# dspcraft/dsc

Measured on AMD Instinct MI355X. Metric: batched 1-D rfft GSamples/s, higher is better.
Workload: dtype f32

## Files before the change

### dsc_amd/csrc/fft_r2c_64k.hip

```cpp
#include "kernels.h"

#include <hip/hip_runtime.h>

#include <cmath>
#include <cstdlib>
#include <utility>

namespace {

typedef float f2 __attribute__((ext_vector_type(2)));

struct cf { float x, y; };
__device__ __forceinline__ cf operator+(cf a, cf b) { return cf{a.x + b.x, a.y + b.y}; }
__device__ __forceinline__ cf operator-(cf a, cf b) { return cf{a.x - b.x, a.y - b.y}; }
__device__ __forceinline__ cf to_cf(f2 a) { return cf{a.x, a.y}; }
__device__ __forceinline__ f2 to_f2(cf a) { return f2{a.x, a.y}; }

constexpr int kM = 32768;
constexpr int kPlaneFloats = 1024 * 34;
constexpr int kLdsBytes = kPlaneFloats * 4 + 1024 * 8;
constexpr int kTabEntries = 1024;

constexpr int kAuxW1024 = 0, kAuxW32768 = 1024, kAuxW65536 = 2048, kAuxEntries = 3072;

__host__ __device__ constexpr int br5(int x) {
    return ((x & 1) << 4) | ((x & 2) << 2) | (x & 4) | ((x & 8) >> 2) | ((x & 16) >> 4);
}

__device__ constexpr float kCos64[17] = {
    1.0f, 0.99518472667219688624f, 0.98078528040323044913f, 0.95694033573220886494f,
    0.92387953251128675613f, 0.88192126434835502971f, 0.83146961230254523708f, 0.77301045336273696081f,
    0.70710678118654752440f, 0.63439328416364549822f, 0.55557023301960222474f, 0.47139673682599764856f,
    0.38268343236508977173f, 0.29028467725446236764f, 0.19509032201612826785f, 0.09801714032956060199f,
    0.0f};

__device__ constexpr float root64_re(int q) {
    q &= 63;
    return q <= 16 ? kCos64[q] : q <= 32 ? -kCos64[32 - q] : q <= 48 ? -kCos64[q - 32] : kCos64[64 - q];
}
__device__ constexpr float root64_im(int q) {
    q &= 63;
    return q <= 16 ? -kCos64[16 - q] : q <= 32 ? -kCos64[q - 16] : q <= 48 ? kCos64[48 - q] : kCos64[q - 48];
}

__device__ __forceinline__ cf cmul(cf a, cf w) {
    return cf{a.x * w.x - a.y * w.y, a.x * w.y + a.y * w.x};
}
__device__ __forceinline__ cf cmul_conj(cf a, cf w) {
    return cf{a.x * w.x + a.y * w.y, a.y * w.x - a.x * w.y};
}

template<bool INV>
__device__ __forceinline__ cf twiddle_mul_second_fused(cf a, cf w) {
    if (INV) return cf{__builtin_fmaf(a.y, w.y, a.x * w.x), __builtin_fmaf(-a.x, w.y, a.y * w.x)};
    return cf{__builtin_fmaf(-a.y, w.y, a.x * w.x), __builtin_fmaf(a.y, w.x, a.x * w.y)};
}

template<bool INV, int M, int K>
__device__ __forceinline__ cf mul_root(cf d) {
    constexpr float c8 = 0.70710678118654752440f;
    if constexpr (K == 0) {
        return d;
    } else if constexpr (4 * K == M) {
        return INV ? cf{-d.y, d.x} : cf{d.y, -d.x};
    } else if constexpr (8 * K == M) {
        return INV ? cf{(d.x - d.y) * c8, (d.x + d.y) * c8} : cf{(d.x + d.y) * c8, (d.y - d.x) * c8};
    } else if constexpr (8 * K == 3 * M) {
        return INV ? cf{-(d.x + d.y) * c8, (d.x - d.y) * c8} : cf{(d.y - d.x) * c8, -(d.x + d.y) * c8};
    } else {
        constexpr float wr = root64_re(K * (64 / M));
        constexpr float wi = INV ? -root64_im(K * (64 / M)) : root64_im(K * (64 / M));
        return cf{d.x * wr - d.y * wi, d.x * wi + d.y * wr};
    }
}

#ifdef DSC_DFT32_DIF
template<bool INV, int M, int G, int... K>
__device__ __forceinline__ void dif_group(cf (&v)[32], std::integer_sequence<int, K...>) {
    (([&] {
         const cf u = v[G + K] + v[G + K + M / 2];
         const cf d = v[G + K] - v[G + K + M / 2];
         v[G + K] = u;
         v[G + K + M / 2] = mul_root<INV, M, K>(d);
     }()),
     ...);
}

template<bool INV, int M, int... G>
__device__ __forceinline__ void dif_stage(cf (&v)[32], std::integer_sequence<int, G...>) {
    (dif_group<INV, M, G * M>(v, std::make_integer_sequence<int, M / 2>{}), ...);
}

template<bool INV>
__device__ __forceinline__ void dft32(cf (&v)[32]) {
    dif_stage<INV, 32>(v, std::make_integer_sequence<int, 1>{});
    dif_stage<INV, 16>(v, std::make_integer_sequence<int, 2>{});
    dif_stage<INV, 8>(v, std::make_integer_sequence<int, 4>{});
    dif_stage<INV, 4>(v, std::make_integer_sequence<int, 8>{});
    dif_stage<INV, 2>(v, std::make_integer_sequence<int, 16>{});
}

template<bool INV>
__device__ __forceinline__ void dft32_head(cf (&v)[32]) {
    dif_stage<INV, 32>(v, std::make_integer_sequence<int, 1>{});
    dif_stage<INV, 16>(v, std::make_integer_sequence<int, 2>{});
}
template<bool INV, int Q>
__device__ __forceinline__ void dft32_quarter(cf (&v)[32]) {
    dif_stage<INV, 8>(v, std::integer_sequence<int, Q>{});
    dif_stage<INV, 4>(v, std::integer_sequence<int, 2 * Q, 2 * Q + 1>{});
    dif_stage<INV, 2>(v, std::integer_sequence<int, 4 * Q, 4 * Q + 1, 4 * Q + 2, 4 * Q + 3>{});
}

#else
constexpr double kCos64d[17] = {
    1.0, 0.99518472667219688624, 0.98078528040323044913, 0.95694033573220886494,
    0.92387953251128675613, 0.88192126434835502971, 0.83146961230254523708, 0.77301045336273696081,
    0.70710678118654752440, 0.63439328416364549822, 0.55557023301960222474, 0.47139673682599764856,
    0.38268343236508977173, 0.29028467725446236764, 0.19509032201612826785, 0.09801714032956060199,
    0.0};

template<bool INV, int E>
__device__ __forceinline__ void dit_butterfly(cf &a, cf &b) {
    if constexpr (E == 0) {
        const cf u = a + b, d = a - b;
        a = u; b = d;
    } else if constexpr (E == 8) {
        const cf u = INV ? cf{a.x - b.y, a.y + b.x} : cf{a.x + b.y, a.y - b.x};
        const cf d = INV ? cf{a.x + b.y, a.y - b.x} : cf{a.x - b.y, a.y + b.x};
        a = u; b = d;
    } else {
        constexpr double c = E <= 8 ? kCos64d[2 * E] : -kCos64d[32 - 2 * E];
        constexpr double sn = (E <= 8 ? kCos64d[16 - 2 * E] : kCos64d[2 * E - 16]);
        constexpr double s = INV ? sn : -sn;
        if constexpr ((c < 0 ? -c : c) >= sn) {
            constexpr float t = (float) (s / c), cc = (float) c;
            float p, q;
            if constexpr (t == 1.0f) { p = b.x - b.y; q = b.y + b.x; }
            else if constexpr (t == -1.0f) { p = b.x + b.y; q = b.y - b.x; }
            else { p = __builtin_fmaf(-t, b.y, b.x); q = __builtin_fmaf(t, b.x, b.y); }
            const cf u = cf{__builtin_fmaf(cc, p, a.x), __builtin_fmaf(cc, q, a.y)};
            const cf d = cf{__builtin_fmaf(-cc, p, a.x), __builtin_fmaf(-cc, q, a.y)};
            a = u; b = d;
        } else {
            constexpr float r = (float) (c / s), ss = (float) s;
            const float pn = __builtin_fmaf(-r, b.x, b.y);
            const float q = __builtin_fmaf(r, b.y, b.x);
            const cf u = cf{__builtin_fmaf(-ss, pn, a.x), __builtin_fmaf(ss, q, a.y)};
            const cf d = cf{__builtin_fmaf(ss, pn, a.x), __builtin_fmaf(-ss, q, a.y)};
            a = u; b = d;
        }
    }
}

constexpr int brev_bits(int x, int bits) {
    int r = 0;
    for (int i = 0; i < bits; ++i) r |= ((x >> i) & 1) << (bits - 1 - i);
    return r;
}

template<bool INV, int S, int G, int... J>
__device__ __forceinline__ void dit_group(cf (&v)[32], std::integer_sequence<int, J...>) {
    constexpr int H = 32 >> S;
    constexpr int E = brev_bits(G, S - 1) * (16 >> (S - 1));
    (dit_butterfly<INV, E>(v[2 * H * G + J], v[2 * H * G + J + H]), ...);
}

template<bool INV, int S, int... G>
__device__ __forceinline__ void dit_stage(cf (&v)[32], std::integer_sequence<int, G...>) {
    (dit_group<INV, S, G>(v, std::make_integer_sequence<int, (32 >> S)>{}), ...);
}

template<bool INV>
__device__ __forceinline__ void dft32(cf (&v)[32]) {
    dit_stage<INV, 1>(v, std::make_integer_sequence<int, 1>{});
    dit_stage<INV, 2>(v, std::make_integer_sequence<int, 2>{});
    dit_stage<INV, 3>(v, std::make_integer_sequence<int, 4>{});
    dit_stage<INV, 4>(v, std::make_integer_sequence<int, 8>{});
    dit_stage<INV, 5>(v, std::make_integer_sequence<int, 16>{});
}

template<bool INV>
__device__ __forceinline__ void dft32_head(cf (&v)[32]) {
    dit_stage<INV, 1>(v, std::make_integer_sequence<int, 1>{});
    dit_stage<INV, 2>(v, std::make_integer_sequence<int, 2>{});
}
template<bool INV, int Q>
__device__ __forceinline__ void dft32_quarter(cf (&v)[32]) {
    dit_stage<INV, 3>(v, std::integer_sequence<int, Q>{});
    dit_stage<INV, 4>(v, std::integer_sequence<int, 2 * Q, 2 * Q + 1>{});
    dit_stage<INV, 5>(v, std::integer_sequence<int, 4 * Q, 4 * Q + 1, 4 * Q + 2, 4 * Q + 3>{});
}
#endif

typedef unsigned int u2 __attribute__((ext_vector_type(2)));
typedef unsigned int u4 __attribute__((ext_vector_type(4)));
typedef float f4 __attribute__((ext_vector_type(4)));

#ifndef DSC_LDS_SPLIT_READS
#define DSC_LDS_SPLIT_READS 1
#endif
__device__ __forceinline__ f2 lds_read_b64(const f2 *p) {
#if DSC_LDS_SPLIT_READS
    return *(const volatile __attribute__((address_space(3))) f2 *) p;
#else
    return *p;
#endif
}

__device__ __forceinline__ void lds_barrier() {
    __builtin_amdgcn_fence(__ATOMIC_RELEASE, "workgroup", "local");
    __builtin_amdgcn_s_barrier();
    __builtin_amdgcn_fence(__ATOMIC_ACQUIRE, "workgroup", "local");
}

__device__ __forceinline__ float bperm(int byte_addr, float x) {
    return __int_as_float(__builtin_amdgcn_ds_bpermute(byte_addr, __float_as_int(x)));
}

__device__ __forceinline__ int column_of(int wave, int lane) {
    int kp = lane < 32 ? 32 * wave + lane : 1024 - 32 * wave - (63 - lane);
    return kp == 1024 ? 512 : kp;
}

#ifdef DSC_R2C64K_PROBE
#define PROBE_ARGS , int io_on
#define PROBE_NULL , 1
#define IO_ON io_on
#else
#define PROBE_ARGS
#define PROBE_NULL
#define IO_ON 1
#endif

__device__ __forceinline__ int thread_id(int wave_sgpr) {
    int zero;
    asm volatile("v_mov_b32 %0, 0" : "=v"(zero));
    const int lane = __builtin_amdgcn_mbcnt_hi(-1, __builtin_amdgcn_mbcnt_lo(-1, zero));
    return (wave_sgpr << 6) | lane;
}

#ifndef DSC_STREAM_AUX
#define DSC_STREAM_AUX 2
#endif
constexpr int kStream = DSC_STREAM_AUX;
__device__ __forceinline__ cf load_c(__amdgpu_buffer_rsrc_t r, int voff, int soff) {
    return to_cf(__builtin_bit_cast(f2, __builtin_amdgcn_raw_buffer_load_b64(r, voff, soff, kStream)));
}
#ifndef DSC_FILTER_EARLY_LOADS
#define DSC_FILTER_EARLY_LOADS 4
#endif
#ifndef DSC_IRFFT_PIN_PASS3
#define DSC_IRFFT_PIN_PASS3 1
#endif
#ifndef DSC_IRFFT_EARLY_PAIRS
#define DSC_IRFFT_EARLY_PAIRS 4
#endif
#ifndef DSC_IRFFT_LOAD_AUX
#define DSC_IRFFT_LOAD_AUX 0
#endif
__device__ __forceinline__ cf load_c_spec(__amdgpu_buffer_rsrc_t r, int voff, int soff) {
    return to_cf(__builtin_bit_cast(f2, __builtin_amdgcn_raw_buffer_load_b64(r, voff, soff, DSC_IRFFT_LOAD_AUX)));
}
__device__ __forceinline__ cf load_c_cached(__amdgpu_buffer_rsrc_t r, int voff, int soff) {
    return to_cf(__builtin_bit_cast(f2, __builtin_amdgcn_raw_buffer_load_b64(r, voff, soff, 0)));
}
template<int POLICY>
__device__ __forceinline__ void store_c(cf a, __amdgpu_buffer_rsrc_t r, int voff, int soff) {
    __builtin_amdgcn_raw_buffer_store_b64(__builtin_bit_cast(u2, to_f2(a)), r, voff, soff, POLICY);
}

__device__ __forceinline__ void fill_twiddle_table(f2 *T, const f2 *aux) {
    const int t = threadIdx.x;
    T[t] = aux[kAuxW1024 + (t >> 5) * (t & 31)];
    __syncthreads();
}

constexpr int kCPitch = 33;
static_assert(512 * kCPitch * 8 <= kPlaneFloats * 4, "the step buffer lives inside the plane");

__host__ __device__ constexpr int class_of(int k) { return (k ^ (k >> 1)) & 1; }
__host__ __device__ constexpr int index_in_class(int k) { return ((k >> 2) << 1) | (k & 1); }
static_assert(class_of(br5(0)) == 0 && class_of(br5(7)) == 0 && class_of(br5(24)) == 0 && class_of(br5(31)) == 0 &&
              class_of(br5(8)) == 1 && class_of(br5(23)) == 1, "class 0 = quarters 0 and 3 of a dft32 output");

__device__ __forceinline__ int reader_column(int t) {
    const int a = t >> 5;
    return (t & 31) | ((((a >> 3) | ((a & 7) << 2))) << 5);
}
__device__ __forceinline__ int spectrum_wave(int wave_sgpr) { return (wave_sgpr >> 2) | ((wave_sgpr & 3) << 2); }

template<int Q>
__device__ __forceinline__ void quarter_write(f2 *buf, int wbase, const cf (&v)[32]) {
    int wbase_hi = wbase + 8 * (32 * kCPitch);
    asm("" : "+v"(wbase_hi));
    f2 *lo8 = buf + wbase;
    f2 *hi8 = buf + wbase_hi;
#pragma unroll
    for (int p = 8 * Q; p < 8 * Q + 8; ++p)
        if (index_in_class(br5(p)) < 8) lo8[index_in_class(br5(p)) * (32 * kCPitch)] = to_f2(v[p]);
#pragma unroll
    for (int p = 8 * Q; p < 8 * Q + 8; ++p)
        if (index_in_class(br5(p)) >= 8) hi8[(index_in_class(br5(p)) - 8) * (32 * kCPitch)] = to_f2(v[p]);
}

__device__ __forceinline__ void step_read(const f2 *buf, int row, cf (&dst)[32]) {
    const f2 *r = buf + __mul24(row, kCPitch);
#pragma unroll
    for (int m = 0; m < 32; ++m) dst[m] = to_cf(lds_read_b64(r + m));
}

__device__ __forceinline__ void pin(cf (&v)[32]) {
#pragma unroll
    for (int p = 0; p < 32; p += 8)
        asm volatile("" : "+v"(v[p].x), "+v"(v[p].y), "+v"(v[p + 1].x), "+v"(v[p + 1].y), "+v"(v[p + 2].x), "+v"(v[p + 2].y), "+v"(v[p + 3].x),
                     "+v"(v[p + 3].y), "+v"(v[p + 4].x), "+v"(v[p + 4].y), "+v"(v[p + 5].x), "+v"(v[p + 5].y), "+v"(v[p + 6].x), "+v"(v[p + 6].y),
                     "+v"(v[p + 7].x), "+v"(v[p + 7].y));
}

template<typename Finish>
__device__ __forceinline__ void exchange(f2 *buf, int wbase, int rclass, int rrow, cf (&src)[32], cf (&dst)[32], Finish finish) {
    pin(src);
    lds_barrier();
    finish(std::integral_constant<int, 0>{});
    quarter_write<0>(buf, wbase, src);
    finish(std::integral_constant<int, 3>{});
    quarter_write<3>(buf, wbase, src);
    lds_barrier();
    cf r[32];
    if (rclass == 0) step_read(buf, rrow, r);
    finish(std::integral_constant<int, 1>{});
    lds_barrier();
    quarter_write<1>(buf, wbase, src);
    finish(std::integral_constant<int, 2>{});
    quarter_write<2>(buf, wbase, src);
    lds_barrier();
    if (rclass != 0) step_read(buf, rrow, r);
#pragma unroll
    for (int m = 0; m < 32; ++m) dst[m] = r[m];
}

struct no_hook { __device__ __forceinline__ void operator()() const {} };

template<bool INV, typename Hook = no_hook>
__device__ __forceinline__ void three_passes(cf (&v)[32], float *plane, const f2 *T, const f2 *aux, int wave_sgpr, int col_wave,
                                             bool mirrored_in, bool mirrored_out, Hook before_pass3 = Hook{}) {
    f2 *buf = (f2 *) plane;
    const int wave_class = ((wave_sgpr >> 2) ^ (wave_sgpr >> 3)) & 1;
    dft32_head<INV>(v);
    cf u[32];
    {
        const int t = thread_id(wave_sgpr);
        const int col = mirrored_in ? column_of(col_wave, t & 63) : t;
        const int hi = col >> 5;
        const f2 *th = T + hi;
        const int rc = reader_column(t);
        exchange(buf, __mul24(col & 31, kCPitch) + hi, wave_class, (index_in_class(rc >> 5) << 5) | (rc & 31), v, u, [&](auto Q) {
            constexpr int kQ = decltype(Q)::value;
            dft32_quarter<INV, kQ>(v);
#pragma unroll
            for (int p = 8 * kQ; p < 8 * kQ + 8; ++p) {
                if (p == 0) continue;
                const cf w = to_cf(th[32 * br5(p)]);
                v[p] = INV ? cmul_conj(v[p], w) : cmul(v[p], w);
            }
        });
    }
    dft32_head<INV>(u);
    {
        const int t = thread_id(wave_sgpr);
        const int rc = reader_column(t);
        const int hi = rc >> 5, lo = rc & 31;
        const cf tw2_base = to_cf(aux[kAuxW32768 + __mul24(hi, lo)]);
        const f2 *tl = T + lo;
        const int col_out = mirrored_out ? column_of(col_wave, t & 63) : rc;
        const int k2 = col_out >> 5;
        const int rclass = mirrored_out ? class_of(k2) : wave_class;
        exchange(buf, __mul24(hi, kCPitch) + lo, rclass, (index_in_class(k2) << 5) | (col_out & 31), u, v, [&](auto Q) {
            constexpr int kQ = decltype(Q)::value;
            dft32_quarter<INV, kQ>(u);
#ifdef DSC_DFT32_DIF
            constexpr bool kSumsOnly = false;
#else
            constexpr bool kSumsOnly = true;
#endif
#pragma unroll
            for (int p = 8 * kQ; p < 8 * kQ + 8; ++p) {
                const cf w = p == 0 ? tw2_base : cmul(tw2_base, to_cf(tl[32 * br5(p)]));
                if (kSumsOnly && p < 4) u[p] = twiddle_mul_second_fused<INV>(u[p], w);
                else u[p] = INV ? cmul_conj(u[p], w) : cmul(u[p], w);
            }
        });
    }
    before_pass3();
    dft32<INV>(v);
}

__device__ __forceinline__ void real_pair(cf p, cf q, cf wq, float hs, cf &out_k, cf &out_mk) {
    const cf s = cf{p.x + q.x, p.y - q.y};
    const cf d = cf{p.x - q.x, p.y + q.y};
    const cf wd = cmul(d, wq);
    out_k = cf{hs * s.x + wd.x, hs * s.y + wd.y};
    out_mk = cf{hs * s.x - wd.x, wd.y - hs * s.y};
}

__device__ __forceinline__ int partner_byte_addr(int wave, int lane) {
    return ((wave == 0 && (lane == 63 || lane == 0)) ? lane : 63 - lane) * 4;
}

#ifndef DSC_R2C64K_HELPERS_ONLY
__global__ __launch_bounds__(1024) void rfft64k_kernel(const float *__restrict__ x, f2 *__restrict__ X, int batch,
                                                       const f2 *__restrict__ aux, int in_pitch, int in_len PROBE_ARGS) {
    extern __shared__ __attribute__((aligned(16))) float lds[];
    float *plane = lds;
    f2 *T = (f2 *) (lds + kPlaneFloats);
    fill_twiddle_table(T, aux);

    const int wave_sgpr = __builtin_amdgcn_readfirstlane(threadIdx.x >> 6);

    cf v[32];
    {
        const int row0 = blockIdx.x;
        const __amdgpu_buffer_rsrc_t r0 = __builtin_amdgcn_make_buffer_rsrc(
            (void *) (x + (size_t) row0 * in_pitch), 0, row0 < batch ? in_len * 4 * IO_ON : 0, 0x00020000);
        const int load_off = thread_id(wave_sgpr) * 8;
#pragma unroll
        for (int j1 = 0; j1 < 32; ++j1) v[j1] = load_c(r0, load_off, j1 * 8192);
    }

    for (int row = blockIdx.x; row < batch; row += gridDim.x) {
        const int next_row = row + gridDim.x;
        const __amdgpu_buffer_rsrc_t rnext = __builtin_amdgcn_make_buffer_rsrc(
            (void *) (x + (size_t) next_row * in_pitch), 0, next_row < batch ? in_len * 4 * IO_ON : 0, 0x00020000);
        const __amdgpu_buffer_rsrc_t rout =
            __builtin_amdgcn_make_buffer_rsrc((void *) (X + (size_t) row * (kM + 1)), 0, (kM + 1) * 8 * IO_ON, 0x00020000);

        const int cw = spectrum_wave(wave_sgpr);
        three_passes<false>(v, plane, T, aux, wave_sgpr, cw, false, true);

        const int t4 = thread_id(wave_sgpr);
        const int lane = t4 & 63, wave = t4 >> 6;
        const int kp = column_of(cw, lane);
        const int partner_addr = partner_byte_addr(cw, lane);
        cf xk[16], xm[16];
        const cf zmid = v[br5(16)];
        if (cw == 0) {
#pragma unroll
            for (int r = 16; r < 31; ++r) v[br5(r)] = lane == 0 ? v[br5(r + 1)] : v[br5(r)];
            v[br5(31)] = lane == 0 ? v[br5(0)] : v[br5(31)];
        }
#pragma unroll
        for (int k3 = 0; k3 < 16; ++k3) {
            const int src = 31 - br5(k3);
            xm[k3].x = bperm(partner_addr, v[src].x);
            xm[k3].y = bperm(partner_addr, v[src].y);
        }
        {
            const cf wpost = to_cf(aux[kAuxW65536 + kp]);
            const cf post_base = cf{0.5f * wpost.y, -0.5f * wpost.x};
#pragma unroll
            for (int k3 = 0; k3 < 16; ++k3) {
                const cf c = cf{root64_re(k3), root64_im(k3)};
                const cf w = k3 == 0 ? post_base : cmul(post_base, c);
                real_pair(v[br5(k3)], xm[k3], w, 0.5f, xk[k3], xm[k3]);
            }
        }

        f2 *stage = (f2 *) plane;
        const int skew = (int) ((((size_t) (X + (size_t) row * (kM + 1))) >> 3) & 15);
        lds_barrier();
#pragma unroll
        for (int k3 = 0; k3 < 16; ++k3) stage[kp + 1024 * k3] = to_f2(xk[k3]);
        const cf xk15 = xk[15];
        const int load_off = thread_id(wave_sgpr) * 8;
#pragma unroll
        for (int j1 = 0; j1 < 16; ++j1) v[j1] = load_c(rnext, load_off, j1 * 8192);
        lds_barrier();
#pragma unroll
        for (int m = 0; m < 8; ++m) {
            const int k = 2 * (t4 + 1024 * m) - skew;
            if (m > 0 || k >= 0) {
                const f2 lo2 = lds_read_b64(stage + k), hi2 = lds_read_b64(stage + k + 1);
                const f4 q = f4{lo2.x, lo2.y, hi2.x, hi2.y};
                __builtin_amdgcn_raw_buffer_store_b128(__builtin_bit_cast(u4, q), rout, k * 8, 0, kStream);
            } else if (m == 0 && k == -1) {
                __builtin_amdgcn_raw_buffer_store_b64(__builtin_bit_cast(u2, stage[0]), rout, 0, 0, kStream);
            }
            if (m & 1) __builtin_amdgcn_sched_barrier(0);
        }
        lds_barrier();
        constexpr int kStage2 = kM / 2 - 16;
#pragma unroll
        for (int k3 = 0; k3 < 16; ++k3) stage[(kM - kStage2) - kp - 1024 * k3] = to_f2(xm[k3]);
        if (kp >= 1009) stage[kp + 15 * 1024 - kStage2] = to_f2(xk15);
        if (t4 == 0) stage[kM / 2 - kStage2] = f2{zmid.x, -zmid.y};
#pragma unroll
        for (int j1 = 16; j1 < 32; ++j1) v[j1] = load_c(rnext, load_off, j1 * 8192);
        lds_barrier();
#pragma unroll
        for (int m = 0; m < 9; ++m) {
            if (m == 8 && wave != 0) break;
            const int k = kM / 2 + 2 * (t4 + 1024 * m) - skew;
            if (m < 8 || k + 1 <= kM) {
                const f2 lo2 = lds_read_b64(stage + k - kStage2), hi2 = lds_read_b64(stage + k + 1 - kStage2);
                const f4 q = f4{lo2.x, lo2.y, hi2.x, hi2.y};
                __builtin_amdgcn_raw_buffer_store_b128(__builtin_bit_cast(u4, q), rout, k * 8, 0, kStream);
            } else if (m == 8 && k == kM) {
                __builtin_amdgcn_raw_buffer_store_b64(__builtin_bit_cast(u2, stage[k - kStage2]), rout, k * 8, 0, kStream);
            }
            if (m & 1) __builtin_amdgcn_sched_barrier(0);
        }
    }
}

#endif

__device__ __forceinline__ void inverse_prepass_direct(cf (&v)[32], cf y_mid, const f2 *aux, int wave_sgpr) {
    constexpr float kScale = 1.0f / (float) kM;
    const int t1 = thread_id(wave_sgpr);
    const int lane = t1 & 63, wave = t1 >> 6;
    const int c = column_of(wave, lane);
    const int partner_addr = partner_byte_addr(wave, lane);
    if (wave == 0 && lane == 0) { v[0].y = 0.f; v[16].y = 0.f; }
    const cf wpre = to_cf(aux[kAuxW65536 + c]);
    const cf wq_base = cf{0.5f * kScale * wpre.y, 0.5f * kScale * wpre.x};
#pragma unroll
    for (int half = 0; half < 2; ++half) {
        cf zm[8];
#pragma unroll
        for (int i = 0; i < 8; ++i) {
            const int a = half * 8 + i;
            const cf cj = cf{root64_re(a), -root64_im(a)};
            const cf wq = a == 0 ? wq_base : cmul(wq_base, cj);
            real_pair(v[a], v[16 + a], wq, 0.5f * kScale, v[a], zm[i]);
        }
#pragma unroll
        for (int i = 0; i < 8; ++i) {
            const int a = half * 8 + i;
            v[16 + a].x = bperm(partner_addr, zm[i].x);
            v[16 + a].y = bperm(partner_addr, zm[i].y);
        }
    }
    cf w[32];
#pragma unroll
    for (int r = 0; r < 16; ++r) { w[r] = v[r]; w[16 + r] = v[31 - r]; }
    if (wave == 0) {
#pragma unroll
        for (int r = 31; r > 16; --r) w[r] = lane == 0 ? w[r - 1] : w[r];
        w[16] = lane == 0 ? cf{kScale * y_mid.x, -kScale * y_mid.y} : w[16];
    }
#pragma unroll
    for (int r = 0; r < 32; ++r) v[r] = w[r];
}

template<typename IssueNext>
__device__ __forceinline__ void staged_time_store(cf (&v)[32], float *plane, __amdgpu_buffer_rsrc_t rout, int wave_sgpr,
                                                  IssueNext issue_next) {
    f2 *stage = (f2 *) plane;
    const int t4 = thread_id(wave_sgpr);
    const int c4 = reader_column(t4);
    lds_barrier();
#pragma unroll
    for (int p = 0; p < 32; p += 2) stage[c4 + 1024 * br5(p)] = to_f2(v[p]);
    issue_next(true);
    lds_barrier();
#pragma unroll
    for (int m = 0; m < 8; ++m) {
        const int k = 2 * (t4 + 1024 * m);
        const f2 lo2 = lds_read_b64(stage + k), hi2 = lds_read_b64(stage + k + 1);
        const f4 q = f4{lo2.x, lo2.y, hi2.x, hi2.y};
        __builtin_amdgcn_raw_buffer_store_b128(__builtin_bit_cast(u4, q), rout, k * 8, 0, kStream);
        if (m & 1) __builtin_amdgcn_sched_barrier(0);
    }
    lds_barrier();
#pragma unroll
    for (int p = 1; p < 32; p += 2) stage[c4 + 1024 * (br5(p) - 16)] = to_f2(v[p]);
    issue_next(false);
    lds_barrier();
#pragma unroll
    for (int m = 0; m < 8; ++m) {
        const int k = 2 * (t4 + 1024 * m);
        const f2 lo2 = lds_read_b64(stage + k), hi2 = lds_read_b64(stage + k + 1);
        const f4 q = f4{lo2.x, lo2.y, hi2.x, hi2.y};
        __builtin_amdgcn_raw_buffer_store_b128(__builtin_bit_cast(u4, q), rout, (kM / 2 + k) * 8, 0, kStream);
        if (m & 1) __builtin_amdgcn_sched_barrier(0);
    }
}

__device__ __forceinline__ void unzip_rows(cf (&v)[32]) {
    cf nxt[32];
#pragma unroll
    for (int a = 0; a < 16; ++a) { nxt[a] = v[2 * a]; nxt[16 + a] = v[2 * a + 1]; }
#pragma unroll
    for (int a = 0; a < 32; ++a) v[a] = nxt[a];
}

#ifndef DSC_R2C64K_HELPERS_ONLY
__global__ __launch_bounds__(1024) void irfft64k_kernel(const f2 *__restrict__ X, float *__restrict__ x, int batch,
                                                        const f2 *__restrict__ aux, int in_pitch, int in_len PROBE_ARGS) {
    extern __shared__ __attribute__((aligned(16))) float lds[];
    float *plane = lds;
    f2 *T = (f2 *) (lds + kPlaneFloats);
    fill_twiddle_table(T, aux);

    const int wave_sgpr = __builtin_amdgcn_readfirstlane(threadIdx.x >> 6);

    cf v[32];
    cf y_mid = cf{0.f, 0.f};
    {
        const int row0 = blockIdx.x;
        const __amdgpu_buffer_rsrc_t r0 = __builtin_amdgcn_make_buffer_rsrc(
            (void *) (X + (size_t) row0 * in_pitch), 0, row0 < batch ? in_len * 8 * IO_ON : 0, 0x00020000);
        const int t0 = thread_id(wave_sgpr);
        const int c = column_of(t0 >> 6, t0 & 63);
        const int pv = (kM - c - 15 * 1024) * 8;
#pragma unroll
        for (int a = 0; a < 16; ++a) {
            v[a] = load_c_spec(r0, c * 8, a * 8192);
            v[16 + a] = load_c_spec(r0, pv, (15 - a) * 8192);
        }
        if (c == 0) y_mid = load_c_spec(r0, (kM / 2) * 8, 0);
    }

    for (int row = blockIdx.x; row < batch; row += gridDim.x) {
        const int next_row = row + gridDim.x;
        const __amdgpu_buffer_rsrc_t rnext = __builtin_amdgcn_make_buffer_rsrc(
            (void *) (X + (size_t) next_row * in_pitch), 0, next_row < batch ? in_len * 8 * IO_ON : 0, 0x00020000);
        const __amdgpu_buffer_rsrc_t rout =
            __builtin_amdgcn_make_buffer_rsrc((void *) (x + (size_t) row * 65536), 0, 65536 * 4 * IO_ON, 0x00020000);

        inverse_prepass_direct(v, y_mid, aux, wave_sgpr);
        constexpr int kEarly = DSC_IRFFT_EARLY_PAIRS;
        cf early[kEarly > 0 ? 2 * kEarly : 1];
        three_passes<true>(v, plane, T, aux, wave_sgpr, wave_sgpr, true, false, [&]() {
            if constexpr (kEarly > 0) {
                const int t3 = thread_id(wave_sgpr);
                const int c3 = column_of(t3 >> 6, t3 & 63);
                const int pv3 = (kM - c3 - 15 * 1024) * 8;
#pragma unroll
                for (int a = 0; a < kEarly; ++a) {
                    early[2 * a] = load_c_spec(rnext, c3 * 8, a * 8192);
                    early[2 * a + 1] = load_c_spec(rnext, pv3, (15 - a) * 8192);
                }
            }
        });

#if DSC_IRFFT_PIN_PASS3
#pragma unroll
        for (int p = 0; p < 32; p += 8)
            asm volatile("" : "+v"(v[p].x), "+v"(v[p].y), "+v"(v[p + 1].x), "+v"(v[p + 1].y), "+v"(v[p + 2].x), "+v"(v[p + 2].y), "+v"(v[p + 3].x),
                         "+v"(v[p + 3].y), "+v"(v[p + 4].x), "+v"(v[p + 4].y), "+v"(v[p + 5].x), "+v"(v[p + 5].y), "+v"(v[p + 6].x), "+v"(v[p + 6].y),
                         "+v"(v[p + 7].x), "+v"(v[p + 7].y));
#endif
        const int t4 = thread_id(wave_sgpr);
        const int c = column_of(t4 >> 6, t4 & 63);
        const int pv = (kM - c - 15 * 1024) * 8;
        staged_time_store(v, plane, rout, wave_sgpr, [&](bool first_half) {
            if (first_half) {
                y_mid = cf{0.f, 0.f};
                if (c == 0) y_mid = load_c_spec(rnext, (kM / 2) * 8, 0);
#pragma unroll
                for (int i = 0; i < 8; ++i) {
                    v[2 * i] = load_c_spec(rnext, c * 8, (kEarly + i) * 8192);
                    v[16 + 2 * i] = load_c_spec(rnext, pv, (15 - kEarly - i) * 8192);
                }
            } else {
#pragma unroll
                for (int i = 0; i < 8 - kEarly; ++i) {
                    v[2 * i + 1] = load_c_spec(rnext, c * 8, (kEarly + 8 + i) * 8192);
                    v[17 + 2 * i] = load_c_spec(rnext, pv, (7 - kEarly - i) * 8192);
                }
            }
        });
        {
            cf nxt[32];
#pragma unroll
            for (int a = 0; a < 16; ++a) {
                if (a < kEarly)          { nxt[a] = early[2 * a];             nxt[16 + a] = early[2 * a + 1]; }
                else if (a < kEarly + 8) { nxt[a] = v[2 * (a - kEarly)];      nxt[16 + a] = v[16 + 2 * (a - kEarly)]; }
                else                     { nxt[a] = v[2 * (a - kEarly - 8) + 1]; nxt[16 + a] = v[17 + 2 * (a - kEarly - 8)]; }
            }
#pragma unroll
            for (int a = 0; a < 32; ++a) v[a] = nxt[a];
        }
    }
}

__global__ __launch_bounds__(1024) void filter64k_kernel(const float *__restrict__ x, const f2 *__restrict__ H,
                                                         float *__restrict__ y, int batch, const f2 *__restrict__ aux, int in_pitch,
                                                         int in_len) {
    extern __shared__ __attribute__((aligned(16))) float lds[];
    float *plane = lds;
    f2 *T = (f2 *) (lds + kPlaneFloats);
    fill_twiddle_table(T, aux);

    const int wave_sgpr = __builtin_amdgcn_readfirstlane(threadIdx.x >> 6);
    const __amdgpu_buffer_rsrc_t rh = __builtin_amdgcn_make_buffer_rsrc((void *) H, 0, (kM + 1) * 8, 0x00020000);
    constexpr float kScale = 1.0f / (float) kM;

    cf v[32];
    {
        const int row0 = blockIdx.x;
        const __amdgpu_buffer_rsrc_t r0 = __builtin_amdgcn_make_buffer_rsrc(
            (void *) (x + (size_t) row0 * in_pitch), 0, row0 < batch ? in_len * 4 : 0, 0x00020000);
        const int load_off = thread_id(wave_sgpr) * 8;
#pragma unroll
        for (int j1 = 0; j1 < 32; ++j1) v[j1] = load_c(r0, load_off, j1 * 8192);
    }
    for (int row = blockIdx.x; row < batch; row += gridDim.x) {
        const int next_row = row + gridDim.x;
        const __amdgpu_buffer_rsrc_t rnext = __builtin_amdgcn_make_buffer_rsrc(
            (void *) (x + (size_t) next_row * in_pitch), 0, next_row < batch ? in_len * 4 : 0, 0x00020000);
        const __amdgpu_buffer_rsrc_t rout =
            __builtin_amdgcn_make_buffer_rsrc((void *) (y + (size_t) row * 65536), 0, 65536 * 4, 0x00020000);
        const int cw = spectrum_wave(wave_sgpr);
        three_passes<false>(v, plane, T, aux, wave_sgpr, cw, false, true);

        {
            const int t1 = thread_id(wave_sgpr);
            const int lane = t1 & 63, wave = cw;
            const int c = column_of(wave, lane);
            const int partner_addr = partner_byte_addr(wave, lane);
            const cf wc = to_cf(aux[kAuxW65536 + c]);
            const cf post_base = cf{0.5f * wc.y, -0.5f * wc.x};
            const cf pre_base = cf{0.5f * kScale * wc.y, 0.5f * kScale * wc.x};
            if (wave == 0) {
                const cf zmid = v[br5(16)];
                const cf hmid = load_c_cached(rh, (kM / 2) * 8, 0);
                const cf pmid = cmul(cf{zmid.x, -zmid.y}, hmid);
                v[br5(16)] = lane == 0 ? cf{kScale * pmid.x, -kScale * pmid.y} : v[br5(16)];
            }
            cf park = v[br5(16)];
            if (wave == 0) {
#pragma unroll
                for (int r = 16; r < 31; ++r) v[br5(r)] = lane == 0 ? v[br5(r + 1)] : v[br5(r)];
                v[br5(31)] = lane == 0 ? v[br5(0)] : v[br5(31)];
            }
#pragma unroll
            for (int part = 0; part < 8; ++part) {
                cf q[2], zm[2];
#pragma unroll
                for (int i = 0; i < 2; ++i) {
                    const int a = part * 2 + i;
                    q[i].x = bperm(partner_addr, v[br5(31 - a)].x);
                    q[i].y = bperm(partner_addr, v[br5(31 - a)].y);
                }
#pragma unroll
                for (int i = 0; i < 2; ++i) {
                    const int a = part * 2 + i;
                    const cf w64 = cf{root64_re(a), root64_im(a)};
                    cf xk, xm;
                    real_pair(v[br5(a)], q[i], a == 0 ? post_base : cmul(post_base, w64), 0.5f, xk, xm);
                    const cf hk = load_c_cached(rh, c * 8, a * 8192);
                    const cf hm = load_c_cached(rh, (kM - 15 * 1024 - c) * 8, (15 - a) * 8192);
                    cf pk = cmul(xk, hk), pm = cmul(xm, hm);
                    if (a == 0) {
                        pk.y = (c == 0) ? 0.f : pk.y;
                        pm.y = (c == 0) ? 0.f : pm.y;
                    }
                    const cf w64c = cf{root64_re(a), -root64_im(a)};
                    real_pair(pk, pm, a == 0 ? pre_base : cmul(pre_base, w64c), 0.5f * kScale, v[br5(a)], zm[i]);
                }
#pragma unroll
                for (int i = 0; i < 2; ++i) {
                    const int a = part * 2 + i;
                    v[br5(31 - a)].x = bperm(partner_addr, zm[i].x);
                    v[br5(31 - a)].y = bperm(partner_addr, zm[i].y);
                }
                __builtin_amdgcn_sched_barrier(0);
            }
            if (wave == 0) {
#pragma unroll
                for (int r = 31; r > 16; --r) v[br5(r)] = lane == 0 ? v[br5(r - 1)] : v[br5(r)];
                v[br5(16)] = lane == 0 ? park : v[br5(16)];
            }
        }
        cf z[32];
#pragma unroll
        for (int r = 0; r < 32; ++r) z[r] = v[br5(r)];
        constexpr int kEarlyX = DSC_FILTER_EARLY_LOADS;
        cf early[kEarlyX > 0 ? kEarlyX : 1];
        three_passes<true>(z, plane, T, aux, wave_sgpr, cw, true, false, [&]() {
            if constexpr (kEarlyX > 0) {
                const int off = thread_id(wave_sgpr) * 8;
#pragma unroll
                for (int j1 = 0; j1 < kEarlyX; ++j1) early[j1] = load_c(rnext, off, j1 * 8192);
            }
        });
        {
            const int load_off = thread_id(wave_sgpr) * 8;
            staged_time_store(z, plane, rout, wave_sgpr, [&](bool first_half) {
                if (first_half) {
#pragma unroll
                    for (int i = 0; i < 16; ++i) z[2 * i] = load_c(rnext, load_off, (kEarlyX + i) * 8192);
                } else {
#pragma unroll
                    for (int i = 0; i < 16 - kEarlyX; ++i) z[2 * i + 1] = load_c(rnext, load_off, (kEarlyX + 16 + i) * 8192);
                }
            });
#pragma unroll
            for (int j1 = 0; j1 < 32; ++j1) v[j1] = j1 < kEarlyX ? early[j1] : j1 < kEarlyX + 16 ? z[2 * (j1 - kEarlyX)] : z[2 * (j1 - kEarlyX - 16) + 1];
        }
    }
}

#endif

}

#ifndef DSC_R2C64K_HELPERS_ONLY
size_t dsc_r2c64k_table_bytes() { return (size_t) kAuxEntries * sizeof(float) * 2; }

void dsc_r2c64k_build_tables(void *host_dst) {
    float *o = (float *) host_dst;
    auto put = [&](int at, long long k, long long n) {
        const long double a = -2.0L * 3.14159265358979323846264338327950288L * (long double) k / (long double) n;
        o[2 * at] = (float) cosl(a);
        o[2 * at + 1] = (float) sinl(a);
    };
    for (int m = 0; m < kTabEntries; ++m) {
        put(kAuxW1024 + m, m, 1024);
        put(kAuxW32768 + m, m, 32768);
        put(kAuxW65536 + m, m, 65536);
    }
    o[2 * (kAuxW1024 + 256)] = 0.f;  o[2 * (kAuxW1024 + 256) + 1] = -1.f;
    o[2 * (kAuxW1024 + 512)] = -1.f; o[2 * (kAuxW1024 + 512) + 1] = 0.f;
    o[2 * (kAuxW1024 + 768)] = 0.f;  o[2 * (kAuxW1024 + 768) + 1] = 1.f;
}

void dsc_launch_rfft64k(const float *x, void *X, int batch, int in_pitch, int in_len, const void *aux, int n_cu, hipStream_t stream) {
    if (batch <= 0) return;
    static unsigned long long attr_devices = 0;
    if (dsc_first_use_on_device(attr_devices)) {
        DSC_KERNEL_CHECK(hipFuncSetAttribute((const void *) rfft64k_kernel, hipFuncAttributeMaxDynamicSharedMemorySize, kLdsBytes));
    }
    const int grid = batch < n_cu ? batch : n_cu;
    DSC_LAUNCH(rfft64k_kernel, dim3(grid), dim3(1024), kLdsBytes, stream, x, (f2 *) X, batch, (const f2 *) aux, in_pitch, in_len PROBE_NULL);
}

void dsc_launch_irfft64k(const void *X, float *x, int batch, int in_pitch, int in_len, const void *aux, int n_cu, hipStream_t stream) {
    if (batch <= 0) return;
    static unsigned long long attr_devices = 0;
    if (dsc_first_use_on_device(attr_devices)) {
        DSC_KERNEL_CHECK(hipFuncSetAttribute((const void *) irfft64k_kernel, hipFuncAttributeMaxDynamicSharedMemorySize, kLdsBytes));
    }
    const int grid = batch < n_cu ? batch : n_cu;
    DSC_LAUNCH(irfft64k_kernel, dim3(grid), dim3(1024), kLdsBytes, stream, (const f2 *) X, x, batch, (const f2 *) aux, in_pitch, in_len PROBE_NULL);
}
void dsc_launch_filter64k(const float *s, const void *H, float *y, int batch, int in_pitch, int in_len, const void *aux, int n_cu,
                          hipStream_t stream) {
    if (batch <= 0) return;
    static unsigned long long attr_devices = 0;
    if (dsc_first_use_on_device(attr_devices)) {
        DSC_KERNEL_CHECK(hipFuncSetAttribute((const void *) filter64k_kernel, hipFuncAttributeMaxDynamicSharedMemorySize, kLdsBytes));
    }
    const int grid = batch < n_cu ? batch : n_cu;
    DSC_LAUNCH(filter64k_kernel, dim3(grid), dim3(1024), kLdsBytes, stream, s, (const f2 *) H, y, batch, (const f2 *) aux, in_pitch, in_len);
}
#endif
```

Before: 674.4.

## Restructure rfft64k post-processing to interleave real-pair math with staged stores

Reorganizes the forward rfft epilogue so the output is staged in two phases by spectral region: the first eight real-pair outputs (both k and mirror halves) are written to LDS and streamed out while the remaining eight real pairs are computed interleaved with the LDS reads and global stores. Next-row prefetch loads go into a separate nx array and are copied into v at the end, and the real-pair computation uses explicit FMAs with a fused twiddle helper. The intent is to overlap ALU work with store traffic and cut one exposed barrier phase, at the cost of higher register pressure (extra 32-entry buffer) and complex boundary handling in the staging layout.

```diff
diff --git a/dsc_amd/csrc/fft_r2c_64k.hip b/dsc_amd/csrc/fft_r2c_64k.hip
--- a/dsc_amd/csrc/fft_r2c_64k.hip
+++ b/dsc_amd/csrc/fft_r2c_64k.hip
@@ -250,6 +250,12 @@
 #ifndef DSC_FILTER_EARLY_LOADS
 #define DSC_FILTER_EARLY_LOADS 4
 #endif
+#ifndef DSC_RFFT_EARLY_LOADS
+#define DSC_RFFT_EARLY_LOADS 16
+#endif
+#ifndef DSC_RFFT_FREE_AFTER_PAIRS
+#define DSC_RFFT_FREE_AFTER_PAIRS 0
+#endif
 #ifndef DSC_IRFFT_PIN_PASS3
 #define DSC_IRFFT_PIN_PASS3 1
 #endif
@@ -404,6 +410,16 @@
     out_mk = cf{hs * s.x - wd.x, wd.y - hs * s.y};
 }
 
+__device__ __forceinline__ void real_pair_forward(cf p, cf q, cf wq, float hs, cf &out_k, cf &out_mk) {
+    const cf s = cf{p.x + q.x, p.y - q.y};
+    const cf d = cf{p.x - q.x, p.y + q.y};
+    const cf wd = cf{__builtin_fmaf(d.x, wq.x, -(d.y * wq.y)), __builtin_fmaf(d.x, wq.y, d.y * wq.x)};
+    out_k = cf{__builtin_fmaf(hs, s.x, wd.x), __builtin_fmaf(hs, s.y, wd.y)};
+    float hx = hs * s.x, hy = hs * s.y;
+    asm("" : "+v"(hx), "+v"(hy));
+    out_mk = cf{hx - wd.x, wd.y - hy};
+}
+
 __device__ __forceinline__ int partner_byte_addr(int wave, int lane) {
     return ((wave == 0 && (lane == 63 || lane == 0)) ? lane : 63 - lane) * 4;
 }
@@ -438,12 +454,25 @@
         const int cw = spectrum_wave(wave_sgpr);
         three_passes<false>(v, plane, T, aux, wave_sgpr, cw, false, true);
 
+        pin(v);
+
+        constexpr int kCutHi = 12288 + 64;
+        constexpr int kStageHi = kM / 2;
+        constexpr int kStage2 = kM / 4 - 16;
+        static_assert(2 * kCutHi - 15 > 3 * kM / 4, "phase 1's upper part holds bins of xm[0..7] only");
+        static_assert(3 * kM / 4 + 1 - kStageHi >= kM / 4, "phase 1: the two parts do not overlap");
+        static_assert(2 * (16 * 1024 + 64) - kStageHi <= kPlaneFloats / 2 && 2 * kCutHi - kStage2 <= kPlaneFloats / 2, "every staging read is inside the plane");
         const int t4 = thread_id(wave_sgpr);
-        const int lane = t4 & 63, wave = t4 >> 6;
+        const int lane = t4 & 63;
         const int kp = column_of(cw, lane);
         const int partner_addr = partner_byte_addr(cw, lane);
+        f2 *stage = (f2 *) plane;
+        const int skew = (int) ((((size_t) (X + (size_t) row * (kM + 1))) >> 3) & 15);
         cf xk[16], xm[16];
         const cf zmid = v[br5(16)];
+#if DSC_RFFT_FREE_AFTER_PAIRS == 0
+        lds_barrier();
+#endif
         if (cw == 0) {
 #pragma unroll
             for (int r = 16; r < 31; ++r) v[br5(r)] = lane == 0 ? v[br5(r + 1)] : v[br5(r)];
@@ -455,61 +484,83 @@
             xm[k3].x = bperm(partner_addr, v[src].x);
             xm[k3].y = bperm(partner_addr, v[src].y);
         }
-        {
-            const cf wpost = to_cf(aux[kAuxW65536 + kp]);
-            const cf post_base = cf{0.5f * wpost.y, -0.5f * wpost.x};
-#pragma unroll
-            for (int k3 = 0; k3 < 16; ++k3) {
+        const cf wpost = to_cf(aux[kAuxW65536 + kp]);
+        const cf post_base = cf{0.5f * wpost.y, -0.5f * wpost.x};
+
+#pragma unroll
+        for (int k3 = 0; k3 < 8; ++k3) {
+#if DSC_RFFT_FREE_AFTER_PAIRS > 0
+            if (k3 == DSC_RFFT_FREE_AFTER_PAIRS) {
+                lds_barrier();
+#pragma unroll
+                for (int q = 0; q < DSC_RFFT_FREE_AFTER_PAIRS; ++q) {
+                    stage[kp + 1024 * q] = to_f2(xk[q]);
+                    stage[(kM - kStageHi) - kp - 1024 * q] = to_f2(xm[q]);
+                }
+            }
+#endif
+            const cf c = cf{root64_re(k3), root64_im(k3)};
+            const cf w = k3 == 0 ? post_base : twiddle_mul_second_fused<false>(post_base, c);
+            real_pair_forward(v[br5(k3)], xm[k3], w, 0.5f, xk[k3], xm[k3]);
+            if (k3 >= DSC_RFFT_FREE_AFTER_PAIRS) {
+                stage[kp + 1024 * k3] = to_f2(xk[k3]);
+                stage[(kM - kStageHi) - kp - 1024 * k3] = to_f2(xm[k3]);
+                __builtin_amdgcn_sched_barrier(0);
+            }
+        }
+        const cf xk7 = xk[7], xm7 = xm[7];
+        cf nx[32];
+#pragma unroll
+        for (int j1 = 0; j1 < DSC_RFFT_EARLY_LOADS; ++j1) nx[j1] = load_c(rnext, t4 * 8, j1 * 8192);
+        lds_barrier();
+        const int hi_step = wave_sgpr == 0 ? 1024 : 0;
+#pragma unroll
+        for (int s = 0; s < 8; ++s) {
+            const int k = 2 * (t4 + (s < 4 ? 1024 * s : 1024 * (8 + s) + hi_step)) - skew;
+            const f2 *src = stage + (s == 0 ? max(k, 0) : s < 4 ? k : k - kStageHi);
+            const f2 lo2 = lds_read_b64(src), hi2 = lds_read_b64(src + 1);
+            {
+                const int k3 = 8 + s;
+                asm volatile("" : "+v"(v[br5(k3)].x), "+v"(v[br5(k3)].y), "+v"(xm[k3].x), "+v"(xm[k3].y));
+                __builtin_amdgcn_sched_barrier(0);
                 const cf c = cf{root64_re(k3), root64_im(k3)};
-                const cf w = k3 == 0 ? post_base : cmul(post_base, c);
-                real_pair(v[br5(k3)], xm[k3], w, 0.5f, xk[k3], xm[k3]);
-            }
-        }
-
-        f2 *stage = (f2 *) plane;
-        const int skew = (int) ((((size_t) (X + (size_t) row * (kM + 1))) >> 3) & 15);
+                const cf w = twiddle_mul_second_fused<false>(post_base, c);
+                real_pair_forward(v[br5(k3)], xm[k3], w, 0.5f, xk[k3], xm[k3]);
+                asm volatile("" : "+v"(xk[k3].x), "+v"(xk[k3].y), "+v"(xm[k3].x), "+v"(xm[k3].y));
+                __builtin_amdgcn_sched_barrier(0);
+            }
+            if (s == 0 ? k >= 0 : s == 7 ? k + 1 <= kM : true) {
+                const u4 q = __builtin_bit_cast(u4, f4{lo2.x, lo2.y, hi2.x, hi2.y});
+                __builtin_amdgcn_raw_buffer_store_b128(q, rout, k * 8, 0, kStream);
+                asm volatile("s_nop 1" : : "v"(q));
+            } else if (s == 0 ? k == -1 : s == 7 ? k == kM : false) {
+                __builtin_amdgcn_raw_buffer_store_b64(__builtin_bit_cast(u2, lo2), rout, max(k, 0) * 8, 0, kStream);
+            }
+            __builtin_amdgcn_sched_barrier(0);
+        }
         lds_barrier();
 #pragma unroll
-        for (int k3 = 0; k3 < 16; ++k3) stage[kp + 1024 * k3] = to_f2(xk[k3]);
-        const cf xk15 = xk[15];
-        const int load_off = thread_id(wave_sgpr) * 8;
-#pragma unroll
-        for (int j1 = 0; j1 < 16; ++j1) v[j1] = load_c(rnext, load_off, j1 * 8192);
+        for (int k3 = 8; k3 < 16; ++k3) {
+            stage[kp + 1024 * k3 - kStage2] = to_f2(xk[k3]);
+            stage[kM - kp - 1024 * k3 - kStage2] = to_f2(xm[k3]);
+        }
+        if (kp >= 1009) stage[kp + 7 * 1024 - kStage2] = to_f2(xk7);
+        if (kp >= 897) stage[kM - kp - 7 * 1024 - kStage2] = to_f2(xm7);
+        if (t4 == 0) stage[kM / 2 - kStage2] = f2{zmid.x, -zmid.y};
+#pragma unroll
+        for (int j1 = DSC_RFFT_EARLY_LOADS; j1 < 32; ++j1) nx[j1] = load_c(rnext, t4 * 8, j1 * 8192);
         lds_barrier();
 #pragma unroll
-        for (int m = 0; m < 8; ++m) {
+        for (int m = 4; m < 13; ++m) {
+            if (m == 12 && wave_sgpr != 0) break;
             const int k = 2 * (t4 + 1024 * m) - skew;
-            if (m > 0 || k >= 0) {
-                const f2 lo2 = lds_read_b64(stage + k), hi2 = lds_read_b64(stage + k + 1);
-                const f4 q = f4{lo2.x, lo2.y, hi2.x, hi2.y};
-                __builtin_amdgcn_raw_buffer_store_b128(__builtin_bit_cast(u4, q), rout, k * 8, 0, kStream);
-            } else if (m == 0 && k == -1) {
-                __builtin_amdgcn_raw_buffer_store_b64(__builtin_bit_cast(u2, stage[0]), rout, 0, 0, kStream);
-            }
+            const f2 lo2 = lds_read_b64(stage + k - kStage2), hi2 = lds_read_b64(stage + k + 1 - kStage2);
+            const f4 q = f4{lo2.x, lo2.y, hi2.x, hi2.y};
+            __builtin_amdgcn_raw_buffer_store_b128(__builtin_bit_cast(u4, q), rout, k * 8, 0, kStream);
             if (m & 1) __builtin_amdgcn_sched_barrier(0);
         }
-        lds_barrier();
-        constexpr int kStage2 = kM / 2 - 16;
-#pragma unroll
-        for (int k3 = 0; k3 < 16; ++k3) stage[(kM - kStage2) - kp - 1024 * k3] = to_f2(xm[k3]);
-        if (kp >= 1009) stage[kp + 15 * 1024 - kStage2] = to_f2(xk15);
-        if (t4 == 0) stage[kM / 2 - kStage2] = f2{zmid.x, -zmid.y};
-#pragma unroll
-        for (int j1 = 16; j1 < 32; ++j1) v[j1] = load_c(rnext, load_off, j1 * 8192);
-        lds_barrier();
-#pragma unroll
-        for (int m = 0; m < 9; ++m) {
-            if (m == 8 && wave != 0) break;
-            const int k = kM / 2 + 2 * (t4 + 1024 * m) - skew;
-            if (m < 8 || k + 1 <= kM) {
-                const f2 lo2 = lds_read_b64(stage + k - kStage2), hi2 = lds_read_b64(stage + k + 1 - kStage2);
-                const f4 q = f4{lo2.x, lo2.y, hi2.x, hi2.y};
-                __builtin_amdgcn_raw_buffer_store_b128(__builtin_bit_cast(u4, q), rout, k * 8, 0, kStream);
-            } else if (m == 8 && k == kM) {
-                __builtin_amdgcn_raw_buffer_store_b64(__builtin_bit_cast(u2, stage[k - kStage2]), rout, k * 8, 0, kStream);
-            }
-            if (m & 1) __builtin_amdgcn_sched_barrier(0);
-        }
+#pragma unroll
+        for (int j1 = 0; j1 < 32; ++j1) v[j1] = nx[j1];
     }
 }
 
```

Result: no change. 671.3 (-0.5%).
